# linghaosong/Sextans

Hardware: AMD Instinct MI355X
Metric: SpMM GFLOP/s + achieved HBM GB/s (fp32, N=16) at 1/2/4/8 MI355X (higher is better)
Workload: dtype f32; 1 GPU; config4: synthetic CSR 4000000x4000000, Poisson(40) nnz/row, U(-1,1) fp32, N=16, alpha=0.85, beta=-2.06, column-major B/C, seed 4; M=4000000, K=4000000, N=16, nnz=159999547, parallelism=1 GPU

## Files before the change

### sextans_amd/csrc/engine.hip

```cpp
#include <algorithm>
#include <cstdlib>
#include <cstring>

#include "engine_launch.h"
#include "window_plan.h"

namespace sxe {
thread_local std::string g_last_error;
}
using namespace sxe;

namespace sxe {

int check_device(int device) {
    int n = 0;
    if (hipGetDeviceCount(&n) != hipSuccess || n <= 0) {
        g_last_error = "hipGetDeviceCount: no HIP device";
        return SEXTANS_ERR_NO_DEVICE;
    }
    if (device < 0 || device >= n) return SEXTANS_ERR_INVALID;
    hipDeviceProp_t p;
    if (hipGetDeviceProperties(&p, device) != hipSuccess) return SEXTANS_ERR_NO_DEVICE;
    if (strncmp(p.gcnArchName, "gfx950", 6) != 0) {
        g_last_error = std::string("device is ") + p.gcnArchName + ", engine is built for gfx950 only";
        return SEXTANS_ERR_NO_DEVICE;
    }
    return SEXTANS_OK;
}

enum Drops { kNothing, kWindowStream, kClusterPlan, kPackedPlans, kColwiseVerdict };
constexpr int64_t kMin = INT64_MIN, kMax = INT64_MAX;
using E = sextans_engine;
static const struct Option {
    const char *key; int64_t E::*slot; Drops drops = kNothing; bool measurement = false; int64_t lo = kMin, hi = kMax; uint64_t only = 0;
} kOptions[] = {
    {"kernel", &E::opt_kernel}, {"stage_a", &E::opt_stage}, {"xcd_remap", &E::opt_xcd}, {"exact", &E::opt_exact}, {"profile", &E::opt_profile},
    {"split_rows", &E::opt_split_rows}, {"bucket_rows", &E::opt_bucket_rows}, {"global_nnz", &E::opt_global_nnz}, {"exact_chain", &E::opt_exact_chain},
    {"fuse_b", &E::opt_fuse_b}, {"small_v2", &E::opt_small_v2}, {"colwise_tiles_adjacent", &E::opt_colwise_tiles_adjacent}, {"window_auto", &E::opt_win_auto},
    {"bell_wide", &E::opt_bell_wide}, {"bell_generation", &E::opt_bell_gen}, {"bell_shared", &E::opt_bell_shared}, {"mfma_dense_tiles", &E::opt_mfma_dense},
    {"dense_tile_fill_x100", &E::opt_dense_fill_x100},
    {"lanes_per_row", &E::opt_lpr, kNothing, false, kMin, kMax, 1 | 1 << 2 | 1 << 4 | 1 << 8},
    {"cols_per_lane", &E::opt_cols_per_lane, kNothing, false, kMin, kMax, 1 | 1 << 4 | 1 << 8},
    {"window_unroll", &E::opt_win_unroll, kNothing, false, kMin, kMax, 1 << 4 | 1 << 8},
    {"tiles_per_wg", &E::opt_tiles_per_wg, kNothing, false, 0, 1024}, {"panel_v2", &E::opt_panel_v2, kNothing, false, -1, 1},
    {"phase_timing", &E::opt_phase_timing, kNothing, true}, {"reordered_xcd", &E::opt_reordered_xcd, kNothing, true}, {"bell_debug", &E::opt_bell_debug, kNothing, true},
    {"dist_broadcast_runs", &E::opt_dist_broadcast_runs, kNothing, true}, {"rowblock_tiles", &E::opt_rb_tiles, kNothing, true},
    {"cluster_shape", &E::opt_cluster_shape, kClusterPlan, true},
    {"cluster_group", &E::opt_cluster_group, kClusterPlan, true, 1, 64},
    {"panel_min_reuse_x100", &E::opt_min_reuse_x100, kClusterPlan}, {"panel_min_reuse_wide_x100", &E::opt_min_reuse_wide_x100, kClusterPlan},
    {"row_cluster", &E::opt_row_cluster, kClusterPlan, false, -1, 2}, {"row_similarity", &E::opt_row_similarity, kClusterPlan, false, -1, 1},
    {"cluster_top", &E::opt_cluster_top, kClusterPlan}, {"small_panel", &E::opt_small_panel, kClusterPlan}, {"row_sets", &E::opt_row_sets, kClusterPlan},
    {"row_offset", &E::opt_row_offset, kClusterPlan}, {"relabel_columns", &E::opt_relabel_columns, kClusterPlan}, {"run_cluster", &E::opt_run_cluster, kClusterPlan},
    {"refine_sweeps", &E::opt_refine_sweeps, kClusterPlan}, {"refine_rows", &E::opt_refine_rows, kClusterPlan},
    {"window_rows", &E::opt_win_rows, kWindowStream, false, 1, sx::kWinMaxRowsPerWave}, {"window_cols", &E::opt_win_cols, kWindowStream, false, 1, 0x7fffffff},
    {"share_index", &E::opt_share_index, kPackedPlans}, {"split_mixed", &E::opt_split_mixed, kPackedPlans},
    {"colwise_max_len", &E::opt_colwise_max_len, kColwiseVerdict},
};

static const Option *find_option(const char *key) {
    for (const Option &o : kOptions)
        if (!strcmp(key, o.key)) return &o;
    return nullptr;
}

int transposed_options(sextans_engine *h, const char *key, int64_t value) {
    auto skip = [](const char *k) { return !strcmp(k, "row_offset") || !strcmp(k, "global_nnz"); };
    if (key) return skip(key) ? SEXTANS_OK : sextans_set_option(h->tr, key, value);
    for (const auto &o : kOptions)
        if (!skip(o.key) && h->tr->*o.slot != h->*o.slot)
            if (int rc = sextans_set_option(h->tr, o.key, h->*o.slot)) return rc;
    h->tr->opt_mode = h->opt_mode;
    return SEXTANS_OK;
}

}

extern "C" {

const char *sextans_last_error(void) { return g_last_error.c_str(); }

int sextans_device_count(int *count) {
    if (!count) return SEXTANS_ERR_INVALID;
    *count = 0;
    int n = 0;
    if (hipGetDeviceCount(&n) != hipSuccess || n <= 0) return SEXTANS_ERR_NO_DEVICE;
    int ok = 0;
    for (int d = 0; d < n; ++d)
        if (check_device(d) == SEXTANS_OK) ++ok;
    *count = ok;
    return ok > 0 ? SEXTANS_OK : SEXTANS_ERR_NO_DEVICE;
}

int sextans_create(sextans_handle_t *out, int device) {
    if (!out) return SEXTANS_ERR_INVALID;
    *out = nullptr;
    if (int rc = check_device(device)) return rc;
    SX_HIP(hipSetDevice(device));
    auto *h = new sextans_engine();
    h->device = device;
    {
        hipDeviceProp_t p;
        if (hipGetDeviceProperties(&p, device) == hipSuccess && p.multiProcessorCount > 0)
            h->num_cus = p.multiProcessorCount;
    }
    preload_device_code();
    *out = h;
    return SEXTANS_OK;
}

int sextans_destroy(sextans_handle_t h) {
    if (!h) return SEXTANS_ERR_INVALID;
    (void)hipSetDevice(h->device);
    free_matrix(h);
    free_bell(h);
    sextans_profile_reset(h);
    if (h->ev_fork) (void)hipEventDestroy(h->ev_fork);
    if (h->ev_join) (void)hipEventDestroy(h->ev_join);
    if (h->aux_stream) (void)hipStreamDestroy(h->aux_stream);
    for (hipEvent_t e : h->dist_events) (void)hipEventDestroy(e);
    if (h->comm_stream) (void)hipStreamDestroy(h->comm_stream);
    if (h->host_stream) (void)hipStreamDestroy(h->host_stream);
    delete h;
    return SEXTANS_OK;
}

int sextans_set_option(sextans_handle_t h, const char *key, int64_t value) {
    if (!h || !key) return SEXTANS_ERR_INVALID;
    if (!strcmp(key, "mode")) {
        if (value != SEXTANS_MODE_STRICT && value != SEXTANS_MODE_FAST) return SEXTANS_ERR_INVALID;
// ... 118 lines not shown
    const int np = dict_cnt[b - 1], nc = dict_cnt[b];
    for (int i = threadIdx.x; i < np; i += 64) {
        const int c = dict[(int64_t)(b - 1) * stride + i];
        unsigned s = ((unsigned)c * 2654435761u) >> 22;
        while (atomicCAS(&tab[s], -1, c) != -1 && tab[s] != c) s = (s + 1) & 1023u;
    }
    __syncthreads();
    unsigned found = 0;
    for (int i = threadIdx.x; i < nc; i += 64) {
        const int c = dict[(int64_t)b * stride + i];
        unsigned s = ((unsigned)c * 2654435761u) >> 22;
        while (tab[s] != -1 && tab[s] != c) s = (s + 1) & 1023u;
        found += tab[s] == c;
    }
    for (int o = 32; o > 0; o >>= 1) found += __shfl_down(found, o);
    if (threadIdx.x == 0) { atomicAdd(&out[0], (unsigned long long)found); atomicAdd(&out[1], (unsigned long long)nc); }
}
int run16_stat(sextans_engine *h, double *value) {
    *value = 0.0;
    if (h->cluster.state <= 0 || !h->cluster.d_slot_row || h->cluster.psc.plan_nblk <= 0) return SEXTANS_OK;
    const int RB = kBlock / 4 * std::max(1, h->cluster.psc.plan_sets);
    std::vector<int> sr((size_t)h->cluster.psc.plan_nblk * RB);
    SX_HIP(hipMemcpy(sr.data(), h->cluster.d_slot_row, sizeof(int) * sr.size(), hipMemcpyDeviceToHost));
    const std::vector<int> &br = h->cluster.psc.h_blk_row;
    if ((int)br.size() != h->cluster.psc.plan_nblk + 1) return SEXTANS_OK;
    int64_t in_runs = 0, slots = 0;
    for (int b = 0; b < h->cluster.psc.plan_nblk; ++b) {
        const int n = br[(size_t)b + 1] - br[(size_t)b];
        const int *r = sr.data() + (size_t)b * RB;
        slots += n;
        for (int i = 0; i < n;) {
            int j = i + 1;
            while (j < n && r[j] == r[j - 1] + 1) ++j;
            if (j - i >= 16) in_runs += j - i;
            i = j;
        }
    }
    *value = slots ? (double)in_runs / (double)slots : 0.0;
    return SEXTANS_OK;
}
int dict_overlap_stat(sextans_engine *h, double *value) {
    const sextans_engine::PanelState &P = h->cluster.state > 0 ? h->cluster.psc : h->ps;
    *value = 0.0;
    if (!P.plan_built || P.plan_nblk < 2 || !P.d_dict || !P.d_dict_ptr) return SEXTANS_OK;
    DevBuf<unsigned long long> d;
    unsigned long long hv[2] = {0, 0};
    SX_HIP(d.alloc(2));
    SX_HIP(hipMemset(d, 0, sizeof hv));
    hipLaunchKernelGGL(dict_overlap, dim3((unsigned)P.plan_nblk - 1), dim3(64), 0, hipStreamPerThread, P.d_dict_ptr, P.d_dict, P.plan_dict_stride, P.plan_nblk, d);
    SX_HIP(hipMemcpy(hv, d, sizeof hv, hipMemcpyDeviceToHost));
    *value = hv[1] ? (double)hv[0] / (double)hv[1] : 0.0;
    return SEXTANS_OK;
}
}
extern "C" {

int sextans_get_stat(sextans_handle_t h, const char *key, double *value) {
    if (!h || !key || !value) return SEXTANS_ERR_INVALID;
    if (h->d_rp) {
        SX_HIP(hipSetDevice(h->device));
        if (int rc = ensure_dense(h)) return rc;
        if (int rc = ensure_split(h)) return rc;
    }
    if (!strcmp(key, "plan_build_s")) *value = h->mat.plan_build_s;
    else if (!strcmp(key, "window_padded_entries")) *value = (double)h->win.padded;
    else if (!strcmp(key, "window_state")) *value = (double)h->win.state;
    else if (!strcmp(key, "reassociated_rows")) *value = (double)h->split.h_split_rows.size();
    else if (!strcmp(key, "piece_path_rows")) *value = (double)(h->split.nhub + h->split.nchain);
    else if (!strcmp(key, "exact_chain_rows")) *value = (double)h->split.nchain;
    else if (!strcmp(key, "chain_threshold")) *value = (double)h->split.chain_T;
    else if (!strcmp(key, "split_threshold")) *value = (double)h->split.T;
    else if (!strcmp(key, "bucket_threshold")) *value = (double)h->split.bucket_L0;
    else if (!strcmp(key, "dense_tiles")) *value = (double)h->dense.tiles;
    else if (!strcmp(key, "dense_tile_fraction")) *value = h->nnz > 0 ? (double)h->dense.nnz / (double)h->nnz : 0.0;
    else if (!strcmp(key, "dense_tiles_on_mfma")) *value = h->dense.W > 0 ? 1.0 : 0.0;
    else if (!strcmp(key, "bell_share")) *value = h->bell_share;
    else if (!strcmp(key, "row_cluster")) *value = (double)h->cluster.state;
    else if (!strcmp(key, "cluster_shared_fraction")) *value = h->cluster.shared;
    else if (!strcmp(key, "cluster_decline")) *value = (double)h->cluster.decline;
    else if (!strcmp(key, "graph_fallbacks")) *value = (double)h->graph_fallbacks;
    else if (!strcmp(key, "cluster_run16_fraction")) return run16_stat(h, value);
    else if (!strcmp(key, "dict_overlap_consecutive")) return dict_overlap_stat(h, value);
    else if (!strcmp(key, "dist_setup_exchanges")) *value = (double)h->dist_exchanges;
    else if (!strcmp(key, "cluster_graph_kind")) *value = (double)h->cluster.graph_kind;
    else if (!strcmp(key, "cluster_runs")) *value = h->cluster.runs ? 1.0 : 0.0;
    else if (!strcmp(key, "pattern_symmetry")) *value = h->cluster.pattern_symmetry;
    else if (!strcmp(key, "col_range_lo")) *value = (double)h->col_lo;
    else if (!strcmp(key, "col_range_hi")) *value = (double)h->col_hi;
    else if (!strcmp(key, "b_rows_repacked")) *value = h->mat.d_touched ? (double)h->mat.touched_segments * 64.0 : (double)(h->col_hi - h->col_lo);
    else if (!strcmp(key, "colwise")) *value = (double)h->cluster.colwise_state;
    else if (!strcmp(key, "mixed_plan")) *value = h->ps.plan_built && h->ps.plan_mixed ? (h->ps.d_rg_skip && h->opt_split_mixed != 0 ? 2.0 : 1.0) : 0.0;
    else if (!strcmp(key, "row_sets")) *value = (double)(h->cluster.state > 0 ? h->cluster.psc.plan_sets : h->ps.plan_sets);
    else if (!strcmp(key, "row_coherence")) *value = h->cluster.row_coherence;
    else if (!strcmp(key, "panel_blocks_clustered")) *value = (double)h->cluster.psc.plan_nblk;
    else if (!strcmp(key, "device_bytes")) *value = (double)device_bytes(h);
    else if (!strcmp(key, "softmax_long_rows")) *value = (double)h->softmax.long_rows;
    else if (!strcmp(key, "value_refreshes")) *value = (double)h->mat.value_refreshes;
    else if (!strcmp(key, "value_refresh_rebuilt")) *value = (double)h->mat.value_refresh_rebuilt;
    else if (!strcmp(key, "bf16_native_calls")) *value = (double)(h->mat.bf16_native_calls + (h->tr ? h->tr->mat.bf16_native_calls : 0));
    else if (!strcmp(key, "bf16_converted_calls")) *value = (double)(h->mat.bf16_converted_calls + (h->tr ? h->tr->mat.bf16_converted_calls : 0));
    else if (!strcmp(key, "transpose_build_s")) *value = h->at.build_s + (h->tr ? h->tr->mat.plan_build_s : 0.0);
    else if (!strcmp(key, "grid_stride_line")) *value = (double)h->cluster_s2;
    else if (!strcmp(key, "grid_stride_plane")) *value = (double)h->cluster_s3;
    else if (!strcmp(key, "panel_rows_natural")) *value = (double)h->plan_total_dict;
    else if (!strcmp(key, "panel_rows_clustered")) *value = (double)h->cluster.total_dict;
    else if (!strcmp(key, "panel_fraction")) *value = h->ps.plan_panel_frac;
    else if (!strcmp(key, "panel_blocks")) *value = (double)h->ps.plan_nblk;
    else if (!strcmp(key, "index_stream_entries")) *value = (double)(h->cluster.state > 0 ? h->cluster.psc.plan_idx_len : h->ps.plan_idx_len);
    else if (!strcmp(key, "value_stream_entries")) *value = (double)(h->cluster.state > 0 ? h->cluster.psc.plan_stream_len : h->ps.plan_stream_len);
    else return SEXTANS_ERR_INVALID;
    return SEXTANS_OK;
}

int sextans_export_plan(sextans_handle_t h, int lanes_per_row, sextans_packed *out) {
    if (!h || !out || (lanes_per_row != 2 && lanes_per_row != 4 && lanes_per_row != 8)) return SEXTANS_ERR_INVALID;
    if (!h->d_rp) return SEXTANS_ERR_STATE;
    SX_HIP(hipSetDevice(h->device));
    if (int rc = ensure_dense(h)) return rc;
    if (int rc = ensure_split(h)) return rc;
    if (int rc = ensure_plan(h, lanes_per_row, true)) return rc;
    if (!h->ps.plan_built) return SEXTANS_ERR_STATE;
    if (int rc = restore_plan_streams(h)) return rc;
    const auto &ps = h->ps;
    const int M = h->M, nblk = ps.plan_nblk, RB = kBlock / lanes_per_row;
    const size_t L = (size_t)ps.plan_stream_len;
    memset(out, 0, sizeof *out);
    out->M = M; out->K = h->K; out->nnz = h->m_nnz; out->lanes_per_row = lanes_per_row; out->nblk = nblk;
    out->stream_len = (int64_t)L; out->max_dict = ps.plan_max_dict; out->nnz_in_panel_blocks = ps.plan_nnz_panel;
    std::vector<int> rp((size_t)M + 1), cnt((size_t)nblk), bd((size_t)nblk * ps.plan_dict_stride);
    SX_HIP(hipMemcpy(rp.data(), h->m_rp, sizeof(int) * rp.size(), hipMemcpyDeviceToHost));
    if (nblk) {
        SX_HIP(hipMemcpy(cnt.data(), ps.d_dict_ptr, sizeof(int) * cnt.size(), hipMemcpyDeviceToHost));
        SX_HIP(hipMemcpy(bd.data(), ps.d_dict, sizeof(int) * bd.size(), hipMemcpyDeviceToHost));
    }
#define SX_HIP_OUT(call) do { if ((call) != hipSuccess) { g_last_error = #call; (void)hipGetLastError(); sextans_packed_free(out); return SEXTANS_ERR_HIP; } } while (0)
    auto alloc = [](size_t bytes) { return calloc(bytes ? bytes : 1, 1); };
    out->blk_row = (int *)alloc(sizeof(int) * ((size_t)nblk + 1));
    out->dict_ptr = (int *)alloc(sizeof(int) * ((size_t)nblk + 1));
    out->row_off = (int *)alloc(sizeof(int) * ((size_t)M + 1));
    out->idx16 = (uint16_t *)alloc(sizeof(uint16_t) * L);
    out->col32 = (int *)alloc(sizeof(int) * L);
    out->val = (float *)alloc(sizeof(float) * L);
    size_t ndict = 0;
    for (int b = 0; b < nblk; ++b) ndict += (size_t)cnt[(size_t)b];
    out->dict = (int *)alloc(sizeof(int) * ndict);
    if (!out->blk_row || !out->dict_ptr || !out->row_off || !out->idx16 || !out->col32 || !out->val || !out->dict) {
        sextans_packed_free(out);
        return SEXTANS_ERR_ALLOC;
    }
    memcpy(out->blk_row, ps.h_blk_row.data(), sizeof(int) * ((size_t)nblk + 1));
    size_t w = 0;
    for (int b = 0; b < nblk; ++b) {
        out->dict_ptr[b] = (int)w;
        for (int i = 0; i < cnt[(size_t)b]; ++i) out->dict[w++] = bd[(size_t)b * ps.plan_dict_stride + (size_t)i];
    }
    out->dict_ptr[nblk] = (int)w;
    for (int r = 0; r < M; ++r) out->row_off[r + 1] = out->row_off[r] + ((rp[(size_t)r + 1] - rp[(size_t)r] + 3) & ~3);
    if (!ps.d_ioff) {
        SX_HIP_OUT(hipMemcpy(out->idx16, ps.d_lidx, sizeof(uint16_t) * L, hipMemcpyDeviceToHost));
    } else {
        std::vector<uint16_t> comp((size_t)ps.plan_idx_len);
        std::vector<int> ioff((size_t)nblk * RB * 2), sinfo((size_t)nblk * RB * 2);
        SX_HIP_OUT(hipMemcpy(comp.data(), ps.d_lidx, sizeof(uint16_t) * comp.size(), hipMemcpyDeviceToHost));
        SX_HIP_OUT(hipMemcpy(ioff.data(), ps.d_ioff, sizeof(int) * ioff.size(), hipMemcpyDeviceToHost));
        SX_HIP_OUT(hipMemcpy(sinfo.data(), ps.d_row_off, sizeof(int) * sinfo.size(), hipMemcpyDeviceToHost));
        const unsigned pad = (unsigned)ps.plan_pad_row * 16u * (unsigned)lanes_per_row;
// ... 111 lines not shown
```

### sextans_amd/csrc/engine_dist.hip

```cpp
#include <dlfcn.h>

#include <algorithm>
#include <cstring>
#include <mutex>

#include "engine_launch.h"

using namespace sxe;

namespace sxe {
namespace {
__global__ __launch_bounds__(256) void position_rows(int nblk, int RB, const int *__restrict__ blk_row, const int *__restrict__ slot_row, int row0, int *__restrict__ out) {
    const int b = blockIdx.x, s = threadIdx.x;
    if (b >= nblk || s >= RB) return;
    const int p0 = blk_row[b], n = blk_row[b + 1] - p0;
    if (s < n) out[p0 + s] = slot_row[(int64_t)b * RB + s] + row0;
}
}

static bool cc_usable(sextans_engine *h, int N, const Tiling &t) {
    return h->cluster.state == 2 && h->cluster.cm_pays && t.W == 16 && N % 16 == 0 && t.segs.size() == 1 && t.segs[0].width == 16 && h->split.nhub == 0 &&
           h->split.nchain == 0 && csr_only(h) && (h->opt_kernel == 0 || h->opt_kernel == 2) && h->d_Cs && h->cluster.d_slot_row &&
           h->d_Cs.size() >= (size_t)(N / 16) * (size_t)h->M * 16 && h->d_Bp.size() >= (size_t)h->K * (size_t)N && h->cluster.psc.plan_sets == 1 &&
           (h->M >= 65536 || h->m_nnz * (int64_t)N >= ((int64_t)24 << 20)) && (int)h->cluster.psc.h_blk_row.size() == h->cluster.psc.plan_nblk + 1;
// ... 103 lines not shown
    if (i < m.y) C[(int64_t)m.x + i + (int64_t)n * ldc] = S[((int64_t)g * N + n) * lmax + i];
}

int exchange(sextans_engine *h, Rccl *r, void *comm, int world, int rank, const int *mine, int n, std::vector<int> &all, int status, hipStream_t s,
             const char *what) {
    ++h->dist_exchanges;
    const size_t per = (size_t)n + 1;
    std::vector<int> me(per, 0), buf(per * (size_t)world, 0);
    for (int i = 0; i < n; ++i) me[(size_t)i] = status ? 0 : mine[i];
    me[(size_t)n] = status;
    DevBuf<int> d;
    SX_HIP(d.alloc(buf.size()));
    hipError_t e0 = hipMemcpyAsync(d + per * (size_t)rank, me.data(), sizeof(int) * per, hipMemcpyHostToDevice, s);
    const int rc = e0 != hipSuccess ? SEXTANS_OK : rccl_check(r->AllGather(d + per * (size_t)rank, d, per, 2 , comm, s), what);
    hipError_t e1 = (rc || e0 != hipSuccess) ? hipSuccess : hipMemcpyAsync(buf.data(), d, sizeof(int) * buf.size(), hipMemcpyDeviceToHost, s);
    hipError_t e2 = hipStreamSynchronize(s);
    d.reset();
    if (rc) return rc;
    SX_HIP(e0);
    SX_HIP(e1);
    SX_HIP(e2);
    bool peer_failed = false;
    all.assign((size_t)n * (size_t)world, 0);
    for (int g = 0; g < world; ++g) {
        peer_failed = peer_failed || buf[per * (size_t)g + (size_t)n] != 0;
        for (int i = 0; i < n; ++i) all[(size_t)g * n + (size_t)i] = buf[per * (size_t)g + (size_t)i];
    }
    if (status) return status;
    if (peer_failed) {
        g_last_error = std::string(what) + ": another rank reported a failure";
        return SEXTANS_ERR_PEER;
    }
    return SEXTANS_OK;
}

struct Partition {
    int64_t M_total = 0;
    int row0 = 0, m_loc = 0, m_max = 0;
    bool equal = true;
};
int read_partition(int world, int rank, const int *row_ranges, int multiple_of, Partition &p) {
    p = Partition();
    for (int g = 0; g < world; ++g) {
        if (row_ranges[2 * g] != (int)p.M_total || row_ranges[2 * g + 1] < row_ranges[2 * g] || (row_ranges[2 * g + 1] % multiple_of)) return SEXTANS_ERR_INVALID;
        p.M_total = row_ranges[2 * g + 1];
        p.m_max = std::max(p.m_max, row_ranges[2 * g + 1] - row_ranges[2 * g]);
        p.equal = p.equal && row_ranges[2 * g + 1] - row_ranges[2 * g] == row_ranges[1] - row_ranges[0];
    }
    p.row0 = row_ranges[2 * rank];
    p.m_loc = row_ranges[2 * rank + 1] - p.row0;
    return SEXTANS_OK;
}

int exchange_nnz(sextans_engine *h, Rccl *r, void *comm, int world, int rank, const int *row_ranges, bool force, int status, hipStream_t s, bool *exchanged) {
    if (!comm) return status;
    std::vector<int> nnz_key(row_ranges, row_ranges + 2 * world);
    nnz_key.push_back(rank);
    if (!force && h->dist_nnz_key == nnz_key) return status;
    const int mine_nz[2] = {(int)(h->nnz & 0x7fffffff), (int)(h->nnz >> 31)};
    std::vector<int> all_nz;
    *exchanged = true;
    if (int rc = exchange(h, r, comm, world, rank, mine_nz, 2, all_nz, status, s, "ncclAllGather(nnz)")) return rc;
    int64_t total = 0;
    for (int g = 0; g < world; ++g) total += (int64_t)all_nz[2 * (size_t)g] + ((int64_t)all_nz[2 * (size_t)g + 1] << 31);
    if (total != h->opt_global_nnz)
        if (int rc = sextans_set_option(h, "global_nnz", total)) return rc;
    h->dist_nnz_key = nnz_key;
    return SEXTANS_OK;
}

int settle(sextans_engine *h, Rccl *r, void *comm, int world, int rank, int status, bool exchanged, hipStream_t s) {
    if (!comm || !exchanged) return status;
    std::vector<int> none;
    const int rc = exchange(h, r, comm, world, rank, nullptr, 0, none, status, s, "ncclAllGather(status)");
    if (rc) { h->dist_cut_key.clear(); h->dist_nnz_key.clear(); }
    return rc;
}

struct CmSetup {
    Partition p;
    std::vector<int64_t> lmax, off;
    int *d_meta = nullptr;
    bool cc = false;
};
int setup_cm(sextans_engine *h, Rccl *r, void *comm, int world, int rank, const int *row_ranges, int N, int &nchunks, hipStream_t s, bool force, CmSetup &out) {
    bool exchanged = false;
    int st = read_partition(world, rank, row_ranges, 1, out.p);
    const Partition &p = out.p;
    if (!st && p.m_loc != h->M) st = SEXTANS_ERR_INVALID;
    if (!st && !h->d_rp) st = SEXTANS_ERR_STATE;
    if (st && !(force && comm)) return st;
    if (!st && world > 1 && h->opt_row_offset != p.row0) st = sextans_set_option(h, "row_offset", p.row0);
    if (nchunks < 1) nchunks = 1;
    if (nchunks > 16) nchunks = 16;
    if (int rc = exchange_nnz(h, r, comm, world, rank, row_ranges, force, st, s, &exchanged)) return rc;
    bool want_cc = false;
    if (nchunks > 1) {
        st = cc_prepare(h, N, &want_cc);
    } else if (h->M > 0) {
        st = prepare(h, N);
    }
    if (want_cc && h->cluster.psc.plan_nblk < nchunks) want_cc = false;
    std::vector<int> key(row_ranges, row_ranges + 2 * world);
    key.push_back(N); key.push_back(nchunks); key.push_back(rank); key.push_back(want_cc ? 1 : 0);
    if (force || h->dist_cut_key != key || st) {
        h->dist_cut_key.clear();
        const size_t need = (size_t)world * (size_t)p.m_max;
        if (!st && want_cc && h->d_dist_rows.size() < need) {
            if (h->d_dist_rows.alloc(need) != hipSuccess) { (void)hipGetLastError(); st = SEXTANS_ERR_HIP; g_last_error = "hipMalloc(row tables) failed"; }
        }
        bool all_cc = want_cc && !st;
        if (comm) {
            const int mine_f = want_cc ? 1 : 0;
            std::vector<int> f;
            exchanged = true;
            if (int rc = exchange(h, r, comm, world, rank, &mine_f, 1, f, st, s, "ncclAllGather(mode)")) return rc;
            for (int g = 0; g < world; ++g) all_cc = all_cc && f[(size_t)g] != 0;
        } else if (st) {
            return st;
        }
        h->dist_cc = all_cc;
        if (all_cc) {
            cc_table(h, p.row0, h->d_dist_rows + (size_t)rank * p.m_max, s);
            if (comm)
                if (int rc = rccl_check(r->AllGather(h->d_dist_rows + (size_t)rank * p.m_max, h->d_dist_rows, (size_t)p.m_max, 2 , comm, s),
                                        "ncclAllGather(row tables)"))
                    return rc;
            ++h->dist_exchanges;
            SX_HIP(hipStreamSynchronize(s));
        }
        std::vector<int> mine((size_t)nchunks + 1, 0);
        mine[(size_t)nchunks] = p.m_loc;
        for (int c = 1; c < nchunks && !st; ++c) {
            if (all_cc) {
                mine[(size_t)c] = h->cluster.psc.h_blk_row[(size_t)((int64_t)h->cluster.psc.plan_nblk * c / nchunks)];
                continue;
            }
            int a = (int)((int64_t)p.m_loc * c / nchunks);
            st = sextans_align_row(h, N, a, &a);
            mine[(size_t)c] = std::min(std::max(a, mine[(size_t)c - 1]), p.m_loc);
        }
        std::vector<int> all;
        if (!comm) {
            if (st) return st;
            all = mine;
        } else {
            exchanged = true;
            if (int rc = exchange(h, r, comm, world, rank, mine.data(), nchunks + 1, all, st, s, "ncclAllGather(cuts)")) return rc;
        }
        for (int g = 0; g < world && !st; ++g) {
            const int len = row_ranges[2 * g + 1] - row_ranges[2 * g];
            const int *cg = all.data() + (size_t)g * (nchunks + 1);
            if (cg[0] != 0 || cg[nchunks] != len) st = SEXTANS_ERR_STATE;
            for (int c = 0; c < nchunks && !st; ++c)
                if (cg[c + 1] < cg[c]) st = SEXTANS_ERR_STATE;
        }
        if (!st) { h->dist_cuts = all; h->dist_cut_key = key; }
    }
    auto workspaces = [&]() -> int {
        auto cut = [&](int g, int c) { return h->dist_cuts[(size_t)g * (nchunks + 1) + (size_t)c]; };
        out.lmax.assign((size_t)nchunks, 1);
        out.off.assign((size_t)nchunks + 1, 0);
        for (int c = 0; c < nchunks; ++c) {
            for (int g = 0; g < world; ++g) out.lmax[(size_t)c] = std::max<int64_t>(out.lmax[(size_t)c], cut(g, c + 1) - cut(g, c));
            out.off[(size_t)c + 1] = out.off[(size_t)c] + (int64_t)world * N * out.lmax[(size_t)c];
        }
        const size_t meta_floats = (size_t)nchunks * (size_t)world * 2;
        if (h->d_stage.size() < (size_t)out.off[(size_t)nchunks] + meta_floats) h->dist_meta_at = nullptr;
        if (int rc = reserve(h->d_stage, (size_t)out.off[(size_t)nchunks] + meta_floats)) return rc;
        if (!h->comm_stream) SX_HIP(hipStreamCreateWithFlags(&h->comm_stream, hipStreamNonBlocking));
        while (h->dist_events.size() < (size_t)nchunks + 1) {
            hipEvent_t e;
            SX_HIP(hipEventCreateWithFlags(&e, hipEventDisableTiming));
            h->dist_events.push_back(e);
        }
        std::vector<int> meta(meta_floats);
        for (int c = 0; c < nchunks; ++c)
            for (int g = 0; g < world; ++g) {
                meta[((size_t)c * world + g) * 2] = row_ranges[2 * g] + cut(g, c);
                meta[((size_t)c * world + g) * 2 + 1] = cut(g, c + 1) - cut(g, c);
            }
        out.d_meta = reinterpret_cast<int *>(h->d_stage + out.off[(size_t)nchunks]);
        if (h->dist_meta != meta || h->dist_meta_at != out.d_meta) {
            SX_HIP(hipMemcpyAsync(out.d_meta, meta.data(), sizeof(int) * meta.size(), hipMemcpyHostToDevice, s));
            ++h->dist_exchanges;
            SX_HIP(hipStreamSynchronize(s));
            h->dist_meta = meta;
            h->dist_meta_at = out.d_meta;
        }
        out.cc = h->dist_cc;
        if (out.cc)
            if (int rc = reserve(h->d_Cfull, (size_t)p.M_total * (size_t)N)) return rc;
        return SEXTANS_OK;
    };
    if (!st) st = workspaces();
    return settle(h, r, comm, world, rank, st, exchanged, s);
}

int setup_rm(sextans_engine *h, Rccl *r, void *comm, int world, int rank, const int *row_ranges, int N, bool packed, hipStream_t s, bool force, Partition &p) {
    bool exchanged = false;
    int st = read_partition(world, rank, row_ranges, 1, p);
    if (!st && p.m_loc != h->M) st = SEXTANS_ERR_INVALID;
    if (!st && !h->d_rp) st = SEXTANS_ERR_STATE;
    if (st && !(force && comm)) return st;
    if (!st && world > 1 && h->opt_row_offset != p.row0) st = sextans_set_option(h, "row_offset", p.row0);
    if (int rc = exchange_nnz(h, r, comm, world, rank, row_ranges, force, st, s, &exchanged)) return rc;
    if (force && h->M > 0)
        st = rm_plan(h, N, s);
    if (!st && packed && comm) {
        st = reserve(h->d_stage, (size_t)p.M_total * (size_t)N);
        h->dist_meta_at = nullptr;
    }
    return settle(h, r, comm, world, rank, st, exchanged || (force && comm), s);
}

struct BellSetup {
    Partition p;
    int64_t lmax = 1;
    size_t slab = 0;
    int *d_meta = nullptr;
};
int setup_bell(sextans_engine *h, Rccl *r, void *comm, int world, int rank, const int *row_ranges, int N, hipStream_t s, bool force, BellSetup &out) {
    int st = read_partition(world, rank, row_ranges, 32, out.p);
    const Partition &p = out.p;
    if (!st && p.m_loc != h->bell.M) st = SEXTANS_ERR_INVALID;
    if (!st && !h->bell.d_bell_Af) st = SEXTANS_ERR_STATE;
    if (st && !(force && comm)) return st;
    auto workspaces = [&]() -> int {
        out.lmax = std::max<int64_t>(1, p.m_max);
        out.slab = (size_t)N * (size_t)out.lmax;
        const size_t meta_floats = (size_t)world * 2;
        if (h->d_stage.size() < (size_t)world * out.slab + meta_floats) h->dist_meta_at = nullptr;
        if (int rc = reserve(h->d_stage, (size_t)world * out.slab + meta_floats)) return rc;
        std::vector<int> meta(meta_floats);
        for (int g = 0; g < world; ++g) { meta[2 * (size_t)g] = row_ranges[2 * g]; meta[2 * (size_t)g + 1] = row_ranges[2 * g + 1] - row_ranges[2 * g]; }
        out.d_meta = reinterpret_cast<int *>(h->d_stage + (size_t)world * out.slab);
        if (h->dist_meta != meta || h->dist_meta_at != out.d_meta) {
            SX_HIP(hipMemcpyAsync(out.d_meta, meta.data(), sizeof(int) * meta.size(), hipMemcpyHostToDevice, s));
            ++h->dist_exchanges;
            SX_HIP(hipStreamSynchronize(s));
            h->dist_meta = meta;
            h->dist_meta_at = out.d_meta;
        }
        return SEXTANS_OK;
    };
    if (!st) st = workspaces();
    return settle(h, r, comm, world, rank, st, force && comm, s);
}

int dist_args_ok(sextans_handle_t h, void *comm, int world, int rank, const int *row_ranges) {
    return h && (comm || world == 1) && world >= 1 && rank >= 0 && rank < world && row_ranges;
}
}

extern "C" {

int sextans_dist_bind_library(const char *path) {
    std::lock_guard<std::mutex> lk(g_bind_mutex);
    if (g_live_comms > 0) {
        g_last_error = "sextans_dist_bind_library: communicators of the current library are still alive";
        return SEXTANS_ERR_STATE;
    }
    g_bind_path = path && *path ? path : "";
    rccl_bind_locked();
    g_bound = true;
    if (!g_r.lib) { g_last_error = g_rccl_error; return SEXTANS_ERR_STATE; }
    return SEXTANS_OK;
}

int sextans_dist_unique_id(char id[128]) {
    if (!id) return SEXTANS_ERR_INVALID;
    Rccl *r = rccl();
    if (!r) return SEXTANS_ERR_STATE;
    return rccl_check(r->GetUniqueId(id), "ncclGetUniqueId");
}

int sextans_dist_comm_init(void **comm, int device, int world, int rank, const char id[128]) {
    if (!comm || !id || world < 1 || rank < 0 || rank >= world) return SEXTANS_ERR_INVALID;
    if (int rc = check_device(device)) return rc;
    Rccl *r = rccl();
    if (!r) return SEXTANS_ERR_STATE;
    SX_HIP(hipSetDevice(device));
    Id128 u;
    memcpy(u.b, id, 128);
    { std::lock_guard<std::mutex> lk(g_bind_mutex); ++g_live_comms; }
    const int rc = rccl_check(r->CommInitRank(comm, world, u, rank), "ncclCommInitRank");
    if (rc) { std::lock_guard<std::mutex> lk(g_bind_mutex); --g_live_comms; }
    return rc;
}

int sextans_dist_comm_destroy(void *comm) {
    Rccl *r = rccl();
    if (!r || !comm) return SEXTANS_ERR_INVALID;
    const int rc = rccl_check(r->CommDestroy(comm), "ncclCommDestroy");
    std::lock_guard<std::mutex> lk(g_bind_mutex);
    if (g_live_comms > 0) --g_live_comms;
    return rc;
}

int sextans_dist_prepare(sextans_handle_t h, void *comm, int world, int rank, const int *row_ranges, int N, int nchunks, int form, void *stream) {
    if (!dist_args_ok(h, comm, world, rank, row_ranges) || N <= 0) return SEXTANS_ERR_INVALID;
    if (form != SEXTANS_DIST_CSR_COLMAJOR && form != SEXTANS_DIST_CSR_ROWMAJOR && form != SEXTANS_DIST_BELL) return SEXTANS_ERR_INVALID;
    if (N % (form == SEXTANS_DIST_BELL ? 32 : 8)) return SEXTANS_ERR_INVALID;
    Rccl *r = comm ? rccl() : nullptr;
    if (comm && !r) return SEXTANS_ERR_STATE;
    SX_HIP(hipSetDevice(h->device));
    hipStream_t s = (hipStream_t)stream;
    if (form == SEXTANS_DIST_CSR_COLMAJOR) {
        CmSetup cs;
        return setup_cm(h, r, comm, world, rank, row_ranges, N, nchunks, s, true, cs);
    }
    if (form == SEXTANS_DIST_CSR_ROWMAJOR) {
        Partition p;
        return setup_rm(h, r, comm, world, rank, row_ranges, N, nchunks < 0, s, true, p);
    }
    BellSetup bs;
    return setup_bell(h, r, comm, world, rank, row_ranges, N, s, true, bs);
}

int sextans_dist_spmm(sextans_handle_t h, void *comm, int world, int rank, const int *row_ranges, int N, float alpha,
                      const float *d_B, int64_t ldb, float beta, const float *d_C_in, int64_t ldc_in, float *d_C_out,
                      int64_t ldc, int nchunks, void *stream) {
    if (!dist_args_ok(h, comm, world, rank, row_ranges) || N <= 0 || (N % 8) || !d_B || !d_C_in || !d_C_out) return SEXTANS_ERR_INVALID;
    if (!h->d_rp) return SEXTANS_ERR_STATE;
    Rccl *r = comm ? rccl() : nullptr;
    if (comm && !r) return SEXTANS_ERR_STATE;
    SX_HIP(hipSetDevice(h->device));
    hipStream_t s = (hipStream_t)stream;
    CmSetup cs;
    if (int rc = setup_cm(h, r, comm, world, rank, row_ranges, N, nchunks, s, false, cs)) return rc;
    const Partition &p = cs.p;
    const int64_t M_total = p.M_total;
    const int row0 = p.row0, m_max = p.m_max;
    if (ldc < M_total || ldc_in < M_total || ldb < h->K) return SEXTANS_ERR_INVALID;
    auto cut = [&](int g, int c) { return h->dist_cuts[(size_t)g * (nchunks + 1) + (size_t)c]; };
    const std::vector<int64_t> &lmax = cs.lmax, &off = cs.off;
    int *d_meta = cs.d_meta;
    const bool cc = cs.cc;
    bool first = true;
    for (int c = 0; c < nchunks; ++c) {
        float *S = h->d_stage + off[(size_t)c];
        const int c0 = cut(rank, c), c1 = cut(rank, c + 1);
        float *mine = S + (size_t)rank * N * lmax[(size_t)c];
        if (cc) {
            if (first) cc_pre(h, N, d_B, ldb, d_C_in + row0, ldc_in, s);
            first = false;
            const int b0 = (int)((int64_t)h->cluster.psc.plan_nblk * c / nchunks), b1 = c + 1 == nchunks ? h->cluster.psc.plan_nblk : (int)((int64_t)h->cluster.psc.plan_nblk * (c + 1) / nchunks);
            if (int rc = cc_chunk(h, N, alpha, beta, b0, b1, h->d_dist_rows + (size_t)rank * m_max, row0, mine, lmax[(size_t)c], s)) return rc;
        } else if (c1 > c0) {
            if (int rc = sextans_spmm_device_rows(h, N, alpha, d_B, ldb, beta, d_C_in + row0 + c0, ldc_in, mine,
                                                  lmax[(size_t)c], c0, c1, first ? 0 : SEXTANS_ROWS_REUSE_B_PANELS, stream))
                return rc;
            first = false;
        }
        SX_HIP(hipEventRecord(h->dist_events[(size_t)c], s));
        SX_HIP(hipStreamWaitEvent(h->comm_stream, h->dist_events[(size_t)c], 0));
        if (comm)
            if (int rc = rccl_check(r->AllGather(mine, S, (size_t)N * (size_t)lmax[(size_t)c], 7 , comm,
                                                 h->comm_stream), "ncclAllGather"))
                return rc;
        if (cc) {
            for (int g = 0; g < world; ++g)
                launch_slab_rows(true, h->d_Cfull, M_total * 16, h->d_dist_rows + (size_t)g * m_max + cut(g, c), 0, cut(g, c + 1) - cut(g, c),
                                 S + (size_t)g * N * lmax[(size_t)c], lmax[(size_t)c] * 16, N / 16, h->comm_stream);
            continue;
        }
        const unsigned gx = (unsigned)((lmax[(size_t)c] + 255) / 256);
        hipLaunchKernelGGL(dist_unpack_slabs, dim3(gx, (unsigned)N, (unsigned)world), dim3(256), 0, h->comm_stream, S,
                           lmax[(size_t)c], N, reinterpret_cast<const int2 *>(d_meta) + (size_t)c * world, d_C_out, ldc);
    }
    if (cc) launch_tiles_to_colmajor(h->d_Cfull, d_C_out, ldc, (int)M_total, 0, N / 16, N, h->comm_stream);
    SX_HIP(hipEventRecord(h->dist_events[(size_t)nchunks], h->comm_stream));
    SX_HIP(hipStreamWaitEvent(s, h->dist_events[(size_t)nchunks], 0));
    SX_HIP(hipGetLastError());
    return SEXTANS_OK;
}

int sextans_dist_spmm_rm(sextans_handle_t h, void *comm, int world, int rank, const int *row_ranges, int N, float alpha, const float *d_B,
                         int64_t ldb, float beta, const float *d_C_in, int64_t ldc_in, float *d_C_out, int64_t ldc, void *stream) {
    if (!dist_args_ok(h, comm, world, rank, row_ranges) || N <= 0 || (N % 8) || !d_B || !d_C_in || !d_C_out || ldb < N || ldc_in < N || ldc < N)
        return SEXTANS_ERR_INVALID;
    if (!h->d_rp) return SEXTANS_ERR_STATE;
    Rccl *r = comm ? rccl() : nullptr;
    if (comm && !r) return SEXTANS_ERR_STATE;
    SX_HIP(hipSetDevice(h->device));
    hipStream_t s = (hipStream_t)stream;
    const bool packed = ldc != N;
    Partition p;
    if (int rc = setup_rm(h, r, comm, world, rank, row_ranges, N, packed, s, false, p)) return rc;
    const int64_t M_total = p.M_total;
    const int row0 = p.row0, m_loc = p.m_loc;
    const bool equal = p.equal && h->opt_dist_broadcast_runs == 0;
    if (comm && !equal && (!r->Broadcast || !r->GroupStart || !r->GroupEnd)) {
        g_last_error = "RCCL library lacks ncclBroadcast / ncclGroupStart / ncclGroupEnd (row ranges of unequal length)";
        return SEXTANS_ERR_STATE;
    }
    if (m_loc > 0)
        if (int rc = sextans_spmm_device_rm(h, N, alpha, d_B, ldb, beta, d_C_in + (int64_t)row0 * ldc_in, ldc_in, d_C_out + (int64_t)row0 * ldc, ldc, stream))
            return rc;
    if (!comm) return SEXTANS_OK;
    float *X = d_C_out;
    if (packed) {
        X = h->d_stage;
        if (m_loc > 0)
            SX_HIP(hipMemcpy2DAsync(X + (int64_t)row0 * N, sizeof(float) * (size_t)N, d_C_out + (int64_t)row0 * ldc, sizeof(float) * (size_t)ldc, sizeof(float) * (size_t)N,
                                    (size_t)m_loc, hipMemcpyDeviceToDevice, s));
    }
    if (equal) {
        const size_t count = (size_t)m_loc * (size_t)N;
        if (int rc = rccl_check(r->AllGather(X + (size_t)rank * count, X, count, 7 , comm, s), "ncclAllGather(row-major C)")) return rc;
    } else {
        if (int rc = rccl_check(r->GroupStart(), "ncclGroupStart")) return rc;
        int rc = SEXTANS_OK;
        for (int g = 0; g < world && rc == SEXTANS_OK; ++g) {
            const size_t count = (size_t)(row_ranges[2 * g + 1] - row_ranges[2 * g]) * (size_t)N;
            float *run = X + (int64_t)row_ranges[2 * g] * N;
            if (count) rc = rccl_check(r->Broadcast(run, run, count, 7 , g, comm, s), "ncclBroadcast(row-major C)");
// ... 40 lines not shown
```

### sextans_amd/csrc/engine_state.h

```cpp
#pragma once
#include <hip/hip_runtime.h>

#include <chrono>
#include <cstdint>
#include <cstdio>
#include <set>
#include <string>
#include <vector>

#include "device_buffer.h"
#include "sextans_amd.h"
#include "thread_stream.h"

namespace sxe {
extern thread_local std::string g_last_error;
}

#define SX_HIP(call)                                                                    \
    do {                                                                                \
        hipError_t e_ = (call);                                                         \
        if (e_ != hipSuccess) {                                                         \
            char buf_[512];                                                             \
            snprintf(buf_, sizeof buf_, "%s failed: %s (%s:%d)", #call,                 \
                     hipGetErrorString(e_), __FILE__, __LINE__);                        \
// ... 150 lines not shown
        int64_t bytes() const { return d_wstream.bytes() + d_wstep0.bytes(); }
    };
    Window win;
    struct DenseTiles {
        int mb = 0, W = 0;
        DevBuf<int> d_dense_col;
        DevBuf<unsigned char> d_dense_Af;
        int64_t tiles = 0, nnz = 0;
        int64_t built_mfma = -2, built_fill = -2;
        int rb_n = 0;
        int64_t rb_groups = 0;
        DevBuf<int> d_rb_row0, d_rb_gptr, d_rb_gcol;
        DevBuf<float> d_rb_A;
        int sb_n = 0;
        int64_t sb_entries = 0;
        DevBuf<int> d_sb_uptr, d_sb_ucol;
        DevBuf<int> d_srp, d_sci;
        DevBuf<float> d_sv;
        int64_t bytes() const {
            return d_dense_col.bytes() + d_dense_Af.bytes() + d_rb_row0.bytes() + d_rb_gptr.bytes() + d_rb_gcol.bytes() + d_rb_A.bytes() + d_sb_uptr.bytes() +
                   d_sb_ucol.bytes() + d_srp.bytes() + d_sci.bytes() + d_sv.bytes();
        }
    };
    DenseTiles dense;
    double dense_share = 0.0;
    int dense_max_union = 0;
    struct Bell {
        int M = 0, K = 0, W = 0;
        const int *d_bell_col = nullptr;
        DevBuf<int> d_bell_col_owned;
        DevBuf<unsigned char> d_bell_Af;
        int64_t bytes() const { return d_bell_col_owned.bytes() + d_bell_Af.bytes(); }
    };
    Bell bell;
    int bell_max_union = 0;
    double bell_share = 0.0;
    DevBuf<unsigned char> d_bell_Bf;
    const int *s_rp = nullptr, *s_ci = nullptr;
    const float *s_v = nullptr;
    int64_t s_nnz = 0;
    const int *m_rp = nullptr, *m_ci = nullptr;
    const float *m_v = nullptr;
    int64_t m_nnz = 0;
    struct PieceTable {
        DevBuf<int> d_vrp, d_vend, d_vfirst, d_row;
        std::vector<int> h_row, h_vfirst;
        int64_t bytes() const { return d_vrp.bytes() + d_vend.bytes() + d_vfirst.bytes() + d_row.bytes(); }
    };
    struct LongRows {
        DevBuf<int> d_mrp, d_mci;
        DevBuf<float> d_mv;
        DevBuf<unsigned char> d_skip;
        PieceTable by_len, by_row;
        int nchain = 0;
        DevBuf<int> d_chain_row, d_chain_beg, d_chain_perm;
        DevBuf<long long> d_chain_off;
        std::vector<int> h_chain_row;
        std::vector<long long> h_chain_off;
        int64_t chain_T = 0;
        int64_t chain_built_opt = -2;
        std::vector<int> h_split_rows;
        int nhub = 0;
        int nv = 0;
        int64_t T = 0, bucket_L0 = 0;
        int64_t built_opt = -2, bucket_built_opt = -2, built_gnnz = -2;
        int64_t bytes() const {
            return d_mrp.bytes() + d_mci.bytes() + d_mv.bytes() + d_skip.bytes() + by_len.bytes() + by_row.bytes() + d_chain_row.bytes() + d_chain_beg.bytes() +
                   d_chain_perm.bytes() + d_chain_off.bytes();
        }
    };
    LongRows split;
    hipStream_t aux_stream = nullptr;
    hipEvent_t ev_fork = nullptr, ev_join = nullptr;
    DevBuf<float> d_P;
    DevBuf<long long> d_dbg;
    DevBuf<float> d_stage;
    int64_t graph_fallbacks = 0;
    hipStream_t comm_stream = nullptr;
    std::vector<hipEvent_t> dist_events;
    DevBuf<float> d_rmB, d_rmC;
    DevBuf<float> d_Cfull;
    DevBuf<int> d_dist_rows;
    bool dist_cc = false;
    int64_t dist_exchanges = 0;
    std::vector<int> dist_nnz_key;
    std::vector<int> dist_cut_key, dist_cuts;
    std::vector<int> dist_meta;
    const int *dist_meta_at = nullptr;
    int64_t workspace_bytes() const {
        return d_Bp.bytes() + d_B.bytes() + d_Cin.bytes() + d_Cout.bytes() + d_chB.bytes() + d_chC.bytes() + d_Cs.bytes() + d_bell_Bf.bytes() + d_P.bytes() +
               d_dbg.bytes() + d_stage.bytes() + d_rmB.bytes() + d_rmC.bytes() + d_Cfull.bytes() + d_dist_rows.bytes();
    }
    int64_t opt_share_index = 1;
    int64_t opt_refine_rows = 62;
    int64_t opt_refine_sweeps = 8;
    int64_t opt_run_cluster = 0;
    int64_t opt_reordered_xcd = -1;
    int64_t opt_row_similarity = -1;
    int64_t opt_relabel_columns = 1;
    int64_t opt_colwise_tiles_adjacent = 1;
    int64_t opt_split_mixed = 1;
    int64_t opt_small_panel = 1;
    int64_t opt_cluster_top = 1 << 30;
    int64_t opt_colwise_max_len = 6;
    int64_t opt_kernel = 0, opt_lpr = 0, opt_stage = 1, opt_xcd = 1, opt_exact = 1, opt_profile = 0;
    int64_t opt_cols_per_lane = 0;
    int64_t opt_cluster_shape = 0;
    int64_t opt_cluster_group = 6;
    int64_t opt_row_cluster = -1;
    int64_t opt_row_offset = -1;
    int64_t opt_row_sets = 2;
    int64_t opt_small_v2 = 1;
    int64_t opt_panel_v2 = -1;
    int64_t opt_tiles_per_wg = 0;
    int64_t opt_fuse_b = 1;
    int64_t opt_split_rows = 0;
    int64_t opt_global_nnz = 0;
    int64_t opt_exact_chain = 1;
    int64_t opt_bucket_rows = -1;
    int64_t opt_phase_timing = 0;
    int64_t opt_min_reuse_x100 = 200;
    int64_t opt_min_reuse_wide_x100 = 150;
    int64_t opt_win_rows = 319;
    int64_t opt_win_cols = 65536;
    int64_t opt_win_unroll = 8;
    int64_t opt_win_auto = 0;
    int64_t opt_bell_shared = -1;
    int64_t opt_rb_tiles = 0;
    int64_t opt_mode = 0;
    int64_t opt_dist_broadcast_runs = 0;
    int64_t opt_bell_debug = 0;
    int64_t opt_bell_gen = 0;
    int64_t opt_bell_wide = 1;
    int64_t opt_mfma_dense = 0;
    int64_t opt_dense_fill_x100 = 50;
    std::vector<sxe::EventPair> ev_kernel, ev_repack, ev_post;
    const char *last_kernel = "none";
    std::string last_kernel_buf;
    sextans_engine *tr = nullptr;
    struct Transposed {
        DevBuf<int> d_trp, d_tci;
        DevBuf<float> d_tv;
        DevBuf<int> d_tperm;
        double build_s = 0.0;
        int64_t bytes() const { return d_trp.bytes() + d_tci.bytes() + d_tv.bytes() + d_tperm.bytes(); }
    };
    Transposed at;
    DevBuf<int> d_sddmm_row0;
    struct Softmax {
        DevBuf<int> d_sm_wrow;
        DevBuf<int2> d_sm_tab;
        DevBuf<float2> d_sm_part;
        int nchunks = 0, long_rows = 0;
        int64_t bytes() const { return d_sm_wrow.bytes() + d_sm_tab.bytes() + d_sm_part.bytes(); }
    };
    Softmax softmax;
};

namespace sxe {

int check_device(int device);
void free_plan(sextans_engine *h);
void free_cluster_plan(sextans_engine *h);
int64_t plan_key(const sextans_engine *h);
int64_t device_bytes(const sextans_engine *h);
void free_window(sextans_engine *h);
void free_bell(sextans_engine *h);
void free_split(sextans_engine *h);
void free_dense(sextans_engine *h);
void free_matrix(sextans_engine *h);
void free_backward(sextans_engine *h);
int validate_matrix(sextans_engine *h);
void free_softmax(sextans_engine *h);
int ensure_softmax_tables(sextans_engine *h, hipStream_t s);
int prepare_transposed(sextans_engine *h, int N, hipStream_t s);
int transposed_options(sextans_engine *h, const char *key, int64_t value);
int allow_big_lds(sextans_engine *h, const void *kern, int bytes);
int read_back_row_ptr(sextans_engine *h, std::vector<int> &rp, int level = 2);
int read_back_entries(sextans_engine *h, std::vector<int> &ci, std::vector<float> &va, int level = 2);
int ensure_plan(sextans_engine *h, int lpr, bool force);
int ensure_cluster_plan(sextans_engine *h);
int restore_plan_streams(sextans_engine *h);
int ensure_colwise(sextans_engine *h);
int ensure_col_range(sextans_engine *h);
int ensure_window(sextans_engine *h, bool force);
bool window_pays(const sextans_engine *h, int N, int64_t padded);
int ensure_split(sextans_engine *h);
int ensure_dense(sextans_engine *h);
int prepare(sextans_engine *h, int N, bool whole = true, Tiling *out = nullptr);
inline bool colwise_wanted(const sextans_engine *h) { return h->opt_kernel == 4 || (h->opt_kernel == 0 && h->cluster.colwise_state == 1); }
inline bool csr_only(const sextans_engine *h) { return h->dense.W == 0 && h->dense.rb_n == 0; }
int launch_dense_tiles(sextans_engine *h, int N, const Operands &o);
int launch_rowblocks(sextans_engine *h, const std::vector<Seg> &plan, const Operands &o, int N, int row_end);
int mark_rowblock_skip(sextans_engine *h);

int rm_plan(sextans_engine *h, int N, hipStream_t s, Tiling *out = nullptr);
int check_rm_bf16_args(sextans_handle_t h, int N, const uint16_t *d_B, int64_t ldb, const void *d_C_in, int64_t ldc_in, void *d_C_out, int64_t ldc, int c_dtype);
int fork_chains(sextans_engine *h, const Operands &o, const std::vector<Seg> &segs, int ch0, int ch1);
void cc_table(sextans_engine *h, int row0, int *d_out, hipStream_t s);

template <class T>
int upload(DevBuf<T> &dst, const std::vector<T> &src) {
    SX_HIP(dst.alloc(src.size()));
    if (!src.empty()) SX_HIP(hipMemcpy(dst, src.data(), sizeof(T) * src.size(), hipMemcpyHostToDevice));
    return SEXTANS_OK;
}

template <class T>
int reserve(DevBuf<T> &buf, size_t n) {
    SX_HIP(buf.reserve(n));
    return SEXTANS_OK;
}

// ... 21 lines not shown
```

Before: 1636 GFLOP/s.

## Exchange distributed SpMM output rows in place via per-column broadcasts

Adds a default-on in-place distributed path. Each rank computes its row chunks straight into the full C output, and the finished runs are shared per column with grouped RCCL broadcasts, or an all-gather for equal single-chunk partitions, on a comm stream overlapped with compute. This avoids packing into a staging buffer and unpacking afterwards. The cost is many small collectives, one per column per rank per chunk, instead of one contiguous exchange. The measured 1-GPU config has no communicator, but it still takes the new path, which calls the row kernel directly into C_out.

```diff
diff --git a/sextans_amd/csrc/engine.hip b/sextans_amd/csrc/engine.hip
--- a/sextans_amd/csrc/engine.hip
+++ b/sextans_amd/csrc/engine.hip
@@ -45,6 +45,7 @@
     {"tiles_per_wg", &E::opt_tiles_per_wg, kNothing, false, 0, 1024}, {"panel_v2", &E::opt_panel_v2, kNothing, false, -1, 1},
     {"phase_timing", &E::opt_phase_timing, kNothing, true}, {"reordered_xcd", &E::opt_reordered_xcd, kNothing, true}, {"bell_debug", &E::opt_bell_debug, kNothing, true},
     {"dist_broadcast_runs", &E::opt_dist_broadcast_runs, kNothing, true}, {"rowblock_tiles", &E::opt_rb_tiles, kNothing, true},
+    {"dist_staged", &E::opt_dist_staged, kNothing, false, 0, 1},
     {"cluster_shape", &E::opt_cluster_shape, kClusterPlan, true},
     {"cluster_group", &E::opt_cluster_group, kClusterPlan, true, 1, 64},
     {"panel_min_reuse_x100", &E::opt_min_reuse_x100, kClusterPlan}, {"panel_min_reuse_wide_x100", &E::opt_min_reuse_wide_x100, kClusterPlan},
@@ -329,6 +330,7 @@
     else if (!strcmp(key, "cluster_run16_fraction")) return run16_stat(h, value);
     else if (!strcmp(key, "dict_overlap_consecutive")) return dict_overlap_stat(h, value);
     else if (!strcmp(key, "dist_setup_exchanges")) *value = (double)h->dist_exchanges;
+    else if (!strcmp(key, "dist_in_place")) *value = h->dist_last_in_place ? 1.0 : 0.0;
     else if (!strcmp(key, "cluster_graph_kind")) *value = (double)h->cluster.graph_kind;
     else if (!strcmp(key, "cluster_runs")) *value = h->cluster.runs ? 1.0 : 0.0;
     else if (!strcmp(key, "pattern_symmetry")) *value = h->cluster.pattern_symmetry;
diff --git a/sextans_amd/csrc/engine_dist.hip b/sextans_amd/csrc/engine_dist.hip
--- a/sextans_amd/csrc/engine_dist.hip
+++ b/sextans_amd/csrc/engine_dist.hip
@@ -209,6 +209,7 @@
     std::vector<int64_t> lmax, off;
     int *d_meta = nullptr;
     bool cc = false;
+    bool in_place = false;
 };
 int setup_cm(sextans_engine *h, Rccl *r, void *comm, int world, int rank, const int *row_ranges, int N, int &nchunks, hipStream_t s, bool force, CmSetup &out) {
     bool exchanged = false;
@@ -228,25 +229,30 @@
         st = prepare(h, N);
     }
     if (want_cc && h->cluster.psc.plan_nblk < nchunks) want_cc = false;
+    const bool can_in_place = h->opt_dist_staged == 0 && (!comm || (r->Broadcast && r->GroupStart && r->GroupEnd));
     std::vector<int> key(row_ranges, row_ranges + 2 * world);
-    key.push_back(N); key.push_back(nchunks); key.push_back(rank); key.push_back(want_cc ? 1 : 0);
+    key.push_back(N); key.push_back(nchunks); key.push_back(rank); key.push_back((want_cc ? 1 : 0) | (can_in_place ? 2 : 0));
     if (force || h->dist_cut_key != key || st) {
         h->dist_cut_key.clear();
         const size_t need = (size_t)world * (size_t)p.m_max;
         if (!st && want_cc && h->d_dist_rows.size() < need) {
             if (h->d_dist_rows.alloc(need) != hipSuccess) { (void)hipGetLastError(); st = SEXTANS_ERR_HIP; g_last_error = "hipMalloc(row tables) failed"; }
         }
-        bool all_cc = want_cc && !st;
+        bool all_cc = want_cc && !st, all_in_place = can_in_place;
         if (comm) {
-            const int mine_f = want_cc ? 1 : 0;
+            const int mine_f = (want_cc ? 1 : 0) | (can_in_place ? 2 : 0);
             std::vector<int> f;
             exchanged = true;
             if (int rc = exchange(h, r, comm, world, rank, &mine_f, 1, f, st, s, "ncclAllGather(mode)")) return rc;
-            for (int g = 0; g < world; ++g) all_cc = all_cc && f[(size_t)g] != 0;
+            for (int g = 0; g < world; ++g) {
+                all_cc = all_cc && (f[(size_t)g] & 1) != 0;
+                all_in_place = all_in_place && (f[(size_t)g] & 2) != 0;
+            }
         } else if (st) {
             return st;
         }
         h->dist_cc = all_cc;
+        h->dist_in_place = all_in_place && !all_cc;
         if (all_cc) {
             cc_table(h, p.row0, h->d_dist_rows + (size_t)rank * p.m_max, s);
             if (comm)
@@ -286,6 +292,14 @@
     }
     auto workspaces = [&]() -> int {
         auto cut = [&](int g, int c) { return h->dist_cuts[(size_t)g * (nchunks + 1) + (size_t)c]; };
+        if (!h->comm_stream) SX_HIP(hipStreamCreateWithFlags(&h->comm_stream, hipStreamNonBlocking));
+        while (h->dist_events.size() < (size_t)nchunks + 1) {
+            hipEvent_t e;
+            SX_HIP(hipEventCreateWithFlags(&e, hipEventDisableTiming));
+            h->dist_events.push_back(e);
+        }
+        out.in_place = h->dist_in_place;
+        if (out.in_place) return SEXTANS_OK;
         out.lmax.assign((size_t)nchunks, 1);
         out.off.assign((size_t)nchunks + 1, 0);
         for (int c = 0; c < nchunks; ++c) {
@@ -295,12 +309,6 @@
         const size_t meta_floats = (size_t)nchunks * (size_t)world * 2;
         if (h->d_stage.size() < (size_t)out.off[(size_t)nchunks] + meta_floats) h->dist_meta_at = nullptr;
         if (int rc = reserve(h->d_stage, (size_t)out.off[(size_t)nchunks] + meta_floats)) return rc;
-        if (!h->comm_stream) SX_HIP(hipStreamCreateWithFlags(&h->comm_stream, hipStreamNonBlocking));
-        while (h->dist_events.size() < (size_t)nchunks + 1) {
-            hipEvent_t e;
-            SX_HIP(hipEventCreateWithFlags(&e, hipEventDisableTiming));
-            h->dist_events.push_back(e);
-        }
         std::vector<int> meta(meta_floats);
         for (int c = 0; c < nchunks; ++c)
             for (int g = 0; g < world; ++g) {
@@ -375,6 +383,53 @@
     return settle(h, r, comm, world, rank, st, force && comm, s);
 }
 
+int dist_spmm_in_place(sextans_engine *h, Rccl *r, void *comm, int world, int rank, const int *row_ranges, const Partition &p, int N, float alpha,
+                       const float *d_B, int64_t ldb, float beta, const float *d_C_in, int64_t ldc_in, float *d_C_out, int64_t ldc, int nchunks,
+                       hipStream_t s) {
+    auto cut = [&](int g, int c) { return h->dist_cuts[(size_t)g * (nchunks + 1) + (size_t)c]; };
+    const bool exchange_runs = comm && world > 1;
+    const bool gather = nchunks == 1 && p.equal;
+    bool first = true, sent = false;
+    for (int c = 0; c < nchunks; ++c) {
+        const int c0 = cut(rank, c), c1 = cut(rank, c + 1);
+        if (c1 > c0) {
+            if (int rc = sextans_spmm_device_rows(h, N, alpha, d_B, ldb, beta, d_C_in + p.row0 + c0, ldc_in, d_C_out + p.row0 + c0, ldc, c0, c1,
+                                                  first ? 0 : SEXTANS_ROWS_REUSE_B_PANELS, (void *)s))
+                return rc;
+            first = false;
+        }
+        bool any = false;
+        for (int g = 0; g < world; ++g) any = any || cut(g, c + 1) > cut(g, c);
+        if (!exchange_runs || !any) continue;
+        SX_HIP(hipEventRecord(h->dist_events[(size_t)c], s));
+        SX_HIP(hipStreamWaitEvent(h->comm_stream, h->dist_events[(size_t)c], 0));
+        if (int rc = rccl_check(r->GroupStart(), "ncclGroupStart")) return rc;
+        int rc = SEXTANS_OK;
+        for (int n = 0; n < N && rc == SEXTANS_OK; ++n) {
+            float *col = d_C_out + (int64_t)n * ldc;
+            if (gather) {
+                rc = rccl_check(r->AllGather(col + (int64_t)rank * p.m_loc, col, (size_t)p.m_loc, 7 , comm, h->comm_stream), "ncclAllGather(C column)");
+                continue;
+            }
+            for (int g = 0; g < world && rc == SEXTANS_OK; ++g) {
+                const int len = cut(g, c + 1) - cut(g, c);
+                float *run = col + row_ranges[2 * g] + cut(g, c);
+                if (len > 0) rc = rccl_check(r->Broadcast(run, run, (size_t)len, 7 , g, comm, h->comm_stream), "ncclBroadcast(C column run)");
+            }
+        }
+        const int rc2 = rccl_check(r->GroupEnd(), "ncclGroupEnd");
+        if (rc) return rc;
+        if (rc2) return rc2;
+        sent = true;
+    }
+    if (sent) {
+        SX_HIP(hipEventRecord(h->dist_events[(size_t)nchunks], h->comm_stream));
+        SX_HIP(hipStreamWaitEvent(s, h->dist_events[(size_t)nchunks], 0));
+    }
+    SX_HIP(hipGetLastError());
+    return SEXTANS_OK;
+}
+
 int dist_args_ok(sextans_handle_t h, void *comm, int world, int rank, const int *row_ranges) {
     return h && (comm || world == 1) && world >= 1 && rank >= 0 && rank < world && row_ranges;
 }
@@ -460,6 +515,8 @@
     const int64_t M_total = p.M_total;
     const int row0 = p.row0, m_max = p.m_max;
     if (ldc < M_total || ldc_in < M_total || ldb < h->K) return SEXTANS_ERR_INVALID;
+    h->dist_last_in_place = cs.in_place;
+    if (cs.in_place) return dist_spmm_in_place(h, r, comm, world, rank, row_ranges, p, N, alpha, d_B, ldb, beta, d_C_in, ldc_in, d_C_out, ldc, nchunks, s);
     auto cut = [&](int g, int c) { return h->dist_cuts[(size_t)g * (nchunks + 1) + (size_t)c]; };
     const std::vector<int64_t> &lmax = cs.lmax, &off = cs.off;
     int *d_meta = cs.d_meta;
diff --git a/sextans_amd/csrc/engine_state.h b/sextans_amd/csrc/engine_state.h
--- a/sextans_amd/csrc/engine_state.h
+++ b/sextans_amd/csrc/engine_state.h
@@ -256,6 +256,8 @@
     DevBuf<float> d_Cfull;
     DevBuf<int> d_dist_rows;
     bool dist_cc = false;
+    bool dist_in_place = false;
+    bool dist_last_in_place = false;
     int64_t dist_exchanges = 0;
     std::vector<int> dist_nnz_key;
     std::vector<int> dist_cut_key, dist_cuts;
@@ -303,6 +305,7 @@
     int64_t opt_rb_tiles = 0;
     int64_t opt_mode = 0;
     int64_t opt_dist_broadcast_runs = 0;
+    int64_t opt_dist_staged = 0;
     int64_t opt_bell_debug = 0;
     int64_t opt_bell_gen = 0;
     int64_t opt_bell_wide = 1;
```

New measurement: 1636 GFLOP/s. No clear change (-0.0%).
